# DRL-Navigation/DDRL4NAV

Measured on AMD Instinct MI355X. Metric: env-steps/sec (whole node) + PPO update ms, Pong 256 envs at 1/2/4/8 GPUs, higher is better.
Workload: dtype f32 (f16x3 MFMA planes, fp32 accumulate)

## Files before the change

ddrl4nav_amd/csrc/engine2.h:

```cpp
#pragma once
#include "kernels.h"

namespace ddrl {

using f32x16 = __attribute__((ext_vector_type(16))) float;
using f4 = __attribute__((ext_vector_type(4))) float;
using f2 = __attribute__((ext_vector_type(2))) float;
__device__ __forceinline__ f4 ld4(const float* p) { return *(const f4*)p; }
__device__ __forceinline__ void st4(float* p, f4 v) { *(f4*)p = v; }
__device__ __forceinline__ f4 zero4() { return (f4){0.0f, 0.0f, 0.0f, 0.0f}; }
typedef __attribute__((address_space(1))) const void gvoid_t;
typedef __attribute__((address_space(3))) void lvoid_t;
__device__ __forceinline__ void ld16_to_lds(const void* uniform_base, uint32_t lane_bytes, float* lds_wave_base) {
  __builtin_amdgcn_global_load_lds((gvoid_t*)((const char*)uniform_base + lane_bytes), (lvoid_t*)lds_wave_base, 16, 0, 0);
}
__device__ __forceinline__ int wave_u() { return __builtin_amdgcn_readfirstlane((int)(threadIdx.x >> 6)); }
template <int NJ>
__device__ __forceinline__ void direct_copy(const void* uniform_base, const uint32_t (&off)[NJ], float* tile, int wave, int tid, int nquads) {
#pragma unroll
  for (int j = 0; j < NJ; ++j)
    if (256 * (j + 1) <= nquads || tid + 256 * j < nquads) ld16_to_lds(uniform_base, off[j], tile + (64 * wave + 256 * j) * 4);
}
template <int N>
__device__ __forceinline__ void wait_vmcnt() {
  asm volatile("s_waitcnt vmcnt(%0)" ::"n"(N) : "memory");
}
__device__ __forceinline__ void rare_path() { asm volatile("; rare path"); }
__device__ __forceinline__ void st1_so(void* uniform_base, uint32_t lane_bytes, float v) {
  *(float*)((char*)uniform_base + lane_bytes) = v;
}

__device__ __forceinline__ float leaky_f(float v) { return __builtin_fmaxf(v, v * LEAKY); }
__device__ __forceinline__ float leaky_bit(unsigned mask, int bit, float g) {
// ... 87 lines not shown
  }
  __syncthreads();
}

template <class Op>
__global__ __launch_bounds__(Op::THREADS, 1) void engine2_kernel(typename Op::Params P) {
  extern __shared__ __attribute__((aligned(16))) float lds2[];
  Op op;
  const int tid = threadIdx.x;
  op.init(P, tid, lds2);
  typename Op::Regs regs;
  f32x16 acc[Op::TM][Op::TN];
#pragma unroll
  for (int i = 0; i < Op::TM; ++i)
#pragma unroll
    for (int j = 0; j < Op::TN; ++j)
#pragma unroll
      for (int r = 0; r < 16; ++r) acc[i][j][r] = 0.0f;

  int kb = op.kb_begin;
  const int kbe = op.kb_end;
  if (kb < kbe) {
    op.fetch(P, kb, regs);
    op.commit(regs, lds2);
    if (kb + 1 < kbe) op.fetch(P, kb + 1, regs);
  }
  __syncthreads();
  for (; kb + 2 < kbe; kb += 2) {
    engine2_step<Op, 0>(op, P, kb, kbe, regs, acc, lds2);
    engine2_step<Op, 1>(op, P, kb + 1, kbe, regs, acc, lds2);
  }
  for (int rbuf = 0; kb < kbe; ++kb, rbuf ^= 1) engine2_step<Op, -1>(op, P, kb, kbe, regs, acc, lds2, rbuf);
  op.epilogue(P, acc, lds2);
}

template <auto Kernel>
inline void lds_limit_once(int bytes) {
  static bool configured = false;
  if (!configured) {
    (void)hipFuncSetAttribute((const void*)Kernel, hipFuncAttributeMaxDynamicSharedMemorySize, bytes);
    configured = true;
  }
}

template <class Op>
inline void launch_engine2(dim3 grid, const typename Op::Params& p, hipStream_t st) {
  constexpr size_t bytes = (size_t)(2 * Op::STAGE) * sizeof(float);
  if (bytes > 64 * 1024) lds_limit_once<engine2_kernel<Op>>((int)bytes);
  hipLaunchKernelGGL(engine2_kernel<Op>, grid, dim3(Op::THREADS), bytes, st, p);
}

__device__ __forceinline__ float lane_swap1(float v) {
  return __int_as_float(__builtin_amdgcn_update_dpp(0, __float_as_int(v), 0xB1, 0xF, 0xF, true));
}

__device__ __forceinline__ int acc_row(int r, int hi) { return (r & 3) + 8 * (r >> 2) + 4 * hi; }

using f16x2_t = __attribute__((ext_vector_type(2))) _Float16;
using h8v = __attribute__((ext_vector_type(8))) _Float16;
constexpr int NPL = 2, NPROD = 3;
using frag8 = h8v;
constexpr int PA[NPROD] = {1, 0, 0}, PB[NPROD] = {0, 1, 0};
using f32x2_t = __attribute__((ext_vector_type(2))) float;
__device__ __forceinline__ void split_planes_c(float x, float y, float scale, unsigned (&p)[NPL]) {
  const f32x2_t xs = {x * scale, y * scale};
  const f16x2_t a = __builtin_convertvector(xs, f16x2_t);
// ... 61 lines not shown
```

ddrl4nav_amd/csrc/fc2.hip:

```cpp
#include "engine2.h"

namespace ddrl {



struct FcFwdB {
  static constexpr int PITCH = 80, PLANE = 128 * PITCH, B_OFF = NPL * PLANE, LDS_BYTES = 2 * NPL * PLANE;
};

template <bool SPLIT>
__global__ __launch_bounds__(256) void fc_fwd_planes_kernel(const float* __restrict__ a3, int64_t a3_es, const unsigned short* __restrict__ wlb,
                                                            const float* __restrict__ amax, const float* __restrict__ params, int64_t bias_off0,
                                                            int64_t bias_off1, float* __restrict__ h, int64_t h_es, int n, int ne, int nsplit,
                                                            float* __restrict__ part, const float* __restrict__ smax, int smax_es) {
  using K = FcFwdB;
  extern __shared__ __attribute__((aligned(16))) char ldsf[];
  const int tid = threadIdx.x, lane = tid & 63, wave = tid >> 6, l31 = lane & 31, hi = lane >> 5;
  const int wr = wave >> 1, wc = wave & 1;
  int bx = blockIdx.x, by = blockIdx.y, bz = blockIdx.z;
  if (!SPLIT && (gridDim.y & 7) == 0) {
    const int lin = bx + 4 * by, xcd = lin & 7, q = lin >> 3;
    bx = q & 3, by = (q >> 2) * 8 + xcd;
  }
  if (SPLIT) {
    const int G = 4 * (int)gridDim.y, nz = (int)gridDim.z, lin = bx + 4 * by + G * bz, full = (nz & ~7) * G;
    int g, m;
    if (lin < full) {
      const int xcd = lin & 7, r = lin >> 3;
      g = (r / G) * 8 + xcd, m = r % G;
    } else {
      const int l2 = lin - full, xcd = l2 & 7, rest = nz & 7;
      if (rest == 4) {
        g = (nz & ~7) + (xcd >> 1), m = (l2 >> 3) * 2 + (xcd & 1);
      } else {
        g = (nz & ~7) + l2 / G, m = l2 % G;
      }
    }
    bz = g, bx = m & 3, by = m >> 2;
  }
  const int e = SPLIT ? bz % ne : bz, split = SPLIT ? bz / ne : 0, n0 = bx * 128, b0 = by * 128;
  float sa = plane_scale(amax[amax_idx(AMAX_A3, e)]), inv = 1.0f / (sa * plane_scale(amax[amax_idx(AMAX_WL, e)]));
  const int k4 = tid & 7, rr = tid >> 3;
  const float* asrc[4];
#pragma unroll
  for (int j = 0; j < 4; ++j) asrc[j] = a3 + e * a3_es + (int64_t)min(b0 + rr + 32 * j, n - 1) * FLAT + k4 * 4;
  const int k8 = tid & 3, cc = tid >> 2;
  const unsigned short* wsrc = wlb + (int64_t)e * PLANE_ROOM * FLAT * FEAT + (int64_t)(n0 + cc) * FLAT + k8 * 8;
  int aA[2], bB[2];
#pragma unroll
  for (int i = 0; i < 2; ++i) aA[i] = (wr * 64 + i * 32 + l31) * K::PITCH + hi * 16;
#pragma unroll
  for (int j = 0; j < 2; ++j) bB[j] = K::B_OFF + (wc * 64 + j * 32 + l31) * K::PITCH + hi * 16;
  constexpr int DEPTH = SPLIT ? 4 : 1;
  f4 ar[DEPTH][4], wrg[DEPTH][2][NPL];
  auto fetch = [&](int kb, int slot) {
#pragma unroll
    for (int j = 0; j < 4; ++j) ar[slot][j] = ld4(asrc[j] + kb * 32);
#pragma unroll
    for (int j = 0; j < 2; ++j)
#pragma unroll
      for (int p = 0; p < NPL; ++p) wrg[slot][j][p] = *(const f4*)(wsrc + (int64_t)p * FLAT * FEAT + (int64_t)j * 64 * FLAT + kb * 32);
  };
  auto commit = [&](int slot) {
#pragma unroll
    for (int j = 0; j < 4; ++j) {
      const f4 v = ar[slot][j];
      unsigned pa[NPL], pb[NPL];
      split_planes_c(v.x, v.y, sa, pa);
      split_planes_c(v.z, v.w, sa, pb);
      char* d = ldsf + (rr + 32 * j) * K::PITCH + k4 * 8;
#pragma unroll
      for (int p = 0; p < NPL; ++p) *(uint2*)(d + p * K::PLANE) = make_uint2(pa[p], pb[p]);
    }
#pragma unroll
    for (int j = 0; j < 2; ++j)
#pragma unroll
      for (int p = 0; p < NPL; ++p) *(f4*)(ldsf + K::B_OFF + p * K::PLANE + (cc + 64 * j) * K::PITCH + k8 * 16) = wrg[slot][j][p];
  };
  f32x16 acc[2][2];
#pragma unroll
  for (int i = 0; i < 2; ++i)
#pragma unroll
    for (int j = 0; j < 2; ++j)
#pragma unroll
      for (int r = 0; r < 16; ++r) acc[i][j][r] = 0.0f;
  auto compute = [&]() {
#pragma unroll
    for (int kg = 0; kg < 2; ++kg) {
      frag8 a[NPL][2], b[NPL][2];
#pragma unroll
      for (int p = 0; p < NPL; ++p) {
#pragma unroll
        for (int i = 0; i < 2; ++i) a[p][i] = *(const frag8*)(ldsf + aA[i] + p * K::PLANE + kg * 32);
#pragma unroll
        for (int j = 0; j < 2; ++j) b[p][j] = *(const frag8*)(ldsf + bB[j] + p * K::PLANE + kg * 32);
      }
#pragma unroll
      for (int t = 0; t < NPROD; ++t)
#pragma unroll
        for (int i = 0; i < 2; ++i)
#pragma unroll
          for (int j = 0; j < 2; ++j) acc[i][j] = mfma_planes(a[PA[t]][i], b[PB[t]][j], acc[i][j]);
    }
  };
  if constexpr (SPLIT) {
    constexpr int PER = (FLAT / 32) / FC_ACT_SPLITS;
    const int kb0 = split * PER;
#pragma unroll
    for (int d = 0; d < DEPTH && d < PER; ++d) fetch(kb0 + d, d);
    if (smax != nullptr) {
      float m = 0.0f;
      for (int i = tid; i < n; i += 256) m = fmaxf(m, smax[e * smax_es + i]);
      m = wave_fmax(m);
      float* red = (float*)ldsf;
      if (lane == 0) red[wave] = m;
      __syncthreads();
      const float a3top = fmaxf(fmaxf(red[0], red[1]), fmaxf(red[2], red[3]));
      __syncthreads();
      sa = plane_scale(a3top), inv = 1.0f / (sa * plane_scale(amax[amax_idx(AMAX_WL, e)]));
    }
    commit(0);
    if (DEPTH < PER) fetch(kb0 + DEPTH, 0);
    __syncthreads();
#pragma unroll
    for (int k = 0; k < PER; ++k) {
      compute();
      __syncthreads();
      if (k + 1 < PER) {
        commit((k + 1) % DEPTH);
        if (k + 1 + DEPTH < PER) fetch(kb0 + k + 1 + DEPTH, (k + 1) % DEPTH);
      }
      __syncthreads();
    }
  } else {
    constexpr int NKB = FLAT / 32;
    fetch(0, 0);
    commit(0);
    fetch(1, 0);
    __syncthreads();
    for (int kb = 0; kb < NKB; ++kb) {
      compute();
      __syncthreads();
      if (kb + 1 < NKB) {
        commit(0);
        if (kb + 2 < NKB) fetch(kb + 2, 0);
      }
      __syncthreads();
    }
  }
#pragma unroll
  for (int j = 0; j < 2; ++j) {
    const int nn = n0 + wc * 64 + j * 32 + l31;
    const float bias = SPLIT ? 0.0f : params[(e ? bias_off1 : bias_off0) + nn];
    float* dst = SPLIT ? part + ((int64_t)split * ENC_SLOTS + e) * n * FEAT : h + e * h_es;
#pragma unroll
    for (int i = 0; i < 2; ++i)
#pragma unroll
      for (int r = 0; r < 16; ++r) {
        const int b = b0 + wr * 64 + i * 32 + acc_row(r, hi);
        if (b < n) dst[(int64_t)b * FEAT + nn] = acc[i][j][r] * inv + bias;
      }
  }
}

void launch_fc_forward(const EncCall& c, bool allow_split, hipStream_t st, bool per_sample_max) {
  const Workspace& w = *c.ws;
  const int nsplit = allow_split ? fc_forward_splits(c.n) : 1;
  ProfRange pr(c.prof, nsplit > 1 ? "FcFwdSplit" : "FcFwd", st);
  {
    lds_limit_once<fc_fwd_planes_kernel<false>>((int)FcFwdB::LDS_BYTES);
    lds_limit_once<fc_fwd_planes_kernel<true>>((int)FcFwdB::LDS_BYTES);
    const dim3 grid(FEAT / 128, (c.n + 127) / 128, c.L->NE * nsplit);
    if (nsplit > 1)
      hipLaunchKernelGGL(fc_fwd_planes_kernel<true>, grid, dim3(256), FcFwdB::LDS_BYTES, st, w.a3, w.es(A3_N), w.wlb, w.amax, c.params,
                         c.L->enc_base[0] + c.L->enc.lb, c.L->enc_base[c.L->NE - 1] + c.L->enc.lb, w.h, w.es(H_N), c.n, c.L->NE, nsplit, w.wpart,
                         per_sample_max ? w.actmax : (const float*)nullptr, ACT_FUSED_MAX);
    else
      hipLaunchKernelGGL(fc_fwd_planes_kernel<false>, grid, dim3(256), FcFwdB::LDS_BYTES, st, w.a3, w.es(A3_N), w.wlb, w.amax, c.params,
                         c.L->enc_base[0] + c.L->enc.lb, c.L->enc_base[c.L->NE - 1] + c.L->enc.lb, w.h, w.es(H_N), c.n, c.L->NE, 1, w.wpart,
                         (const float*)nullptr, 0);
  }
}

struct FcDgradB {
  static constexpr int KBK = 32, WPE = 2, PITCH = 2 * KBK + 16, PLANE = 128 * PITCH, B_OFF = NPL * PLANE, LDS_BYTES = 2 * NPL * PLANE;
  static constexpr int NAQ = KBK / 4, ARJ = 128 * NAQ / 256, AROWS = 256 / NAQ;
  static constexpr int NWF = KBK / 8, WJ = 128 * NWF / 256, WCOLS = 256 / NWF;
};
__global__ __launch_bounds__(256) __attribute__((amdgpu_waves_per_eu(FcDgradB::WPE, FcDgradB::WPE))) void fc_dgrad_planes_kernel(const float* __restrict__ dh, int64_t dh_es, const unsigned short* __restrict__ wdlb,
                                                              float* __restrict__ amax, const unsigned* __restrict__ m3, float* __restrict__ dz3, int64_t a3_es, int n) {
  using K = FcDgradB;
  extern __shared__ __attribute__((aligned(16))) char ldsg[];
  const int tid = threadIdx.x, lane = tid & 63, wave = tid >> 6, l31 = lane & 31, hi = lane >> 5;
  const int wr = wave >> 1, wc = wave & 1;
  int bx = blockIdx.x, by = blockIdx.y;
  if ((gridDim.y & 7) == 0) {
    const int lin = bx + 25 * by, xcd = lin & 7, q = lin >> 3;
    if ((gridDim.y & 63) != 0) {
      bx = q % 25, by = (q / 25) * 8 + xcd;
    } else {
      const int blk = q / 40, r = q % 40;
      bx = (blk % 5) * 5 + r % 5, by = ((blk / 5) * 8 + r / 5) * 8 + xcd;
    }
  }
  const int e = blockIdx.z, k0 = bx * 128, b0 = by * 128;
  const float sa = plane_scale(amax[amax_idx(AMAX_DH, e)]), inv = 1.0f / (sa * plane_scale(amax[amax_idx(AMAX_WL, e)]));
  const int n4 = tid % K::NAQ, rr = tid / K::NAQ;
  const float* asrc[K::ARJ];
#pragma unroll
  for (int j = 0; j < K::ARJ; ++j) asrc[j] = dh + e * dh_es + (int64_t)min(b0 + rr + K::AROWS * j, n - 1) * FEAT + n4 * 4;
  const int n8 = tid % K::NWF, cc = tid / K::NWF;
  const unsigned short* wsrc[K::WJ];
#pragma unroll
  for (int j = 0; j < K::WJ; ++j) wsrc[j] = wdlb + (int64_t)e * PLANE_ROOM * FLAT * FEAT + (int64_t)min(k0 + cc + K::WCOLS * j, FLAT - 1) * FEAT + n8 * 8;
  int aA[2], bB[2];
#pragma unroll
  for (int i = 0; i < 2; ++i) aA[i] = (wr * 64 + i * 32 + l31) * K::PITCH + hi * 16;
#pragma unroll
  for (int j = 0; j < 2; ++j) bB[j] = K::B_OFF + (wc * 64 + j * 32 + l31) * K::PITCH + hi * 16;
  f4 ar[K::ARJ], wrg[K::WJ][NPL];
  auto fetch = [&](int kb) {
#pragma unroll
    for (int j = 0; j < K::ARJ; ++j) ar[j] = ld4(asrc[j] + kb * K::KBK);
#pragma unroll
    for (int j = 0; j < K::WJ; ++j)
#pragma unroll
      for (int p = 0; p < NPL; ++p) wrg[j][p] = *(const f4*)(wsrc[j] + (int64_t)p * FLAT * FEAT + kb * K::KBK);
  };
  auto commit = [&]() {
#pragma unroll
    for (int j = 0; j < K::ARJ; ++j) {
      const f4 v = ar[j];
      unsigned pa[NPL], pb[NPL];
      split_planes_c(v.x, v.y, sa, pa);
      split_planes_c(v.z, v.w, sa, pb);
      char* d = ldsg + (rr + K::AROWS * j) * K::PITCH + n4 * 8;
#pragma unroll
      for (int p = 0; p < NPL; ++p) *(uint2*)(d + p * K::PLANE) = make_uint2(pa[p], pb[p]);
    }
#pragma unroll
    for (int j = 0; j < K::WJ; ++j)
#pragma unroll
      for (int p = 0; p < NPL; ++p) *(f4*)(ldsg + K::B_OFF + p * K::PLANE + (cc + K::WCOLS * j) * K::PITCH + n8 * 16) = wrg[j][p];
  };
  f32x16 acc[2][2];
#pragma unroll
  for (int i = 0; i < 2; ++i)
#pragma unroll
    for (int j = 0; j < 2; ++j)
#pragma unroll
      for (int r = 0; r < 16; ++r) acc[i][j][r] = 0.0f;
  constexpr int NKB = FEAT / K::KBK;
  fetch(0);
  commit();
  fetch(1);
  __syncthreads();
  for (int kb = 0; kb < NKB; ++kb) {
#pragma unroll
    for (int kg = 0; kg < K::KBK / 16; ++kg) {
      frag8 a[NPL][2], b[NPL][2];
#pragma unroll
      for (int p = 0; p < NPL; ++p) {
#pragma unroll
        for (int i = 0; i < 2; ++i) a[p][i] = *(const frag8*)(ldsg + aA[i] + p * K::PLANE + kg * 32);
#pragma unroll
        for (int j = 0; j < 2; ++j) b[p][j] = *(const frag8*)(ldsg + bB[j] + p * K::PLANE + kg * 32);
      }
#pragma unroll
      for (int t = 0; t < NPROD; ++t)
#pragma unroll
        for (int i = 0; i < 2; ++i)
#pragma unroll
          for (int j = 0; j < 2; ++j) acc[i][j] = mfma_planes(a[PA[t]][i], b[PB[t]][j], acc[i][j]);
    }
    __syncthreads();
    if (kb + 1 < NKB) {
      commit();
      if (kb + 2 < NKB) fetch(kb + 2);
    }
    __syncthreads();
  }
  float big = 0.0f;
#pragma unroll
  for (int j = 0; j < 2; ++j) {
    const int k = k0 + wc * 64 + j * 32 + l31;
    if (k >= FLAT) continue;
    const int ch = k / 49, pix = k % 49;
    const int mbit = 16 * (ch >> 5) + 15 - ((ch & 3) + 4 * ((ch & 31) >> 3));
    const unsigned* mp = m3 + (int64_t)e * (a3_es / A3_N) * M3_N + pix * 2 + ((ch >> 2) & 1);
#pragma unroll
    for (int i = 0; i < 2; ++i) {
      unsigned mw[16];
#pragma unroll
      for (int r = 0; r < 16; ++r) {
        const int b = min(b0 + wr * 64 + i * 32 + acc_row(r, hi), n - 1);
        mw[r] = mp[(int64_t)b * M3_N];
      }
#pragma unroll
      for (int r = 0; r < 16; ++r) {
        const int b = b0 + wr * 64 + i * 32 + acc_row(r, hi);
        const float g = leaky_bit(mw[r], mbit, acc[i][j][r] * inv);
        if (b < n) {
          dz3[e * a3_es + (int64_t)b * FLAT + k] = g;
          big = fmaxf(big, fabsf(g));
        }
      }
    }
  }
  amax_update(big, amax + amax_idx(AMAX_DZ3, e));
}

struct FcWgradB {
  static constexpr int KB = 32, PITCH = 320, PLANE = KB * PITCH, B_OFF = NPL * PLANE, LDS_BYTES = 2 * NPL * PLANE;
  static constexpr int64_t SLAB = SLAB_FC;
};

__global__ __launch_bounds__(256) void fc_wgrad_planes_kernel(const float* __restrict__ dh, int64_t dh_es, const float* __restrict__ a3,
                                                              int64_t a3_es, const float* __restrict__ amax, const float* __restrict__ gsc,
                                                              int64_t gsc_es, float* __restrict__ part, int n, int nsplit, int ne) {
  using K = FcWgradB;
  extern __shared__ __attribute__((aligned(16))) char ldsw[];
  const int tid = threadIdx.x, lane = tid & 63, wave = tid >> 6, l31 = lane & 31, hi = lane >> 5;
  const int wr = wave >> 1, wc = wave & 1;
  const int unit = (int)(blockIdx.x >> 5) * 8 + (int)(blockIdx.x & 7);
  if (unit >= 25 * ne * nsplit) return;
  const int bx = unit % 25, by = (int)(blockIdx.x >> 3) & 3, bz = unit / 25;
  const int e = bz % ne, split = bz / ne;
  const float sd = WGRAD_HEADROOM * plane_scale(amax[amax_idx(AMAX_DH, e)]) / amax[amax_idx(AMAX_GMAX, e)], sa = plane_scale(amax[amax_idx(AMAX_A3, e)]),
              inv = 1.0f / (sd * sa);
  const float* gs = gsc + e * gsc_es;
  const int k0 = bx * 128, n0 = by * 128;
  const int nkb = (n + K::KB - 1) / K::KB;
  const int per = (nkb + nsplit - 1) / nsplit;
  const int kb_begin = split * per, kb_end = min(nkb, kb_begin + per);
  const int c4 = tid & 31, kk = tid >> 5;
  const float* dsrc = dh + e * dh_es + n0 + c4 * 4;
  const float* asrc = a3 + e * a3_es + min(k0 + c4 * 4, FLAT - 4);
  const int g16 = lane >> 4, q = (lane >> 2) & 3, pp = lane & 3;
  int aA[2], bB[2];
#pragma unroll
  for (int i = 0; i < 2; ++i) aA[i] = (8 * (g16 >> 1) + q) * K::PITCH + (wr * 64 + i * 32 + 16 * (g16 & 1) + 4 * pp) * 2;
#pragma unroll
  for (int j = 0; j < 2; ++j) bB[j] = K::B_OFF + (8 * (g16 >> 1) + q) * K::PITCH + (wc * 64 + j * 32 + 16 * (g16 & 1) + 4 * pp) * 2;
  f4 dr[4], ar[4];
  float gr[4];
  f4 bsum = zero4();
  const bool bias_owner = (bx == 0);
  auto fetch = [&](int kb) {
#pragma unroll
    for (int j = 0; j < 4; ++j) {
      const int64_t row = min(kb * K::KB + kk + 8 * j, n - 1);
      dr[j] = ld4(dsrc + row * FEAT);
      ar[j] = ld4(asrc + row * FLAT);
      gr[j] = gs[row];
    }
  };
  auto commit = [&](int kb) {
    if (kb * K::KB + K::KB > n) {
      rare_path();
#pragma unroll
      for (int j = 0; j < 4; ++j)
        if (kb * K::KB + kk + 8 * j >= n) dr[j] = zero4();
      rare_path();
    }
#pragma unroll
    for (int j = 0; j < 4; ++j) {
      char* d = ldsw + (kk + 8 * j) * K::PITCH + c4 * 8;
      unsigned pa[NPL], pb[NPL];
      const float sdj = sd * gr[j];
      split_planes(dr[j].x, dr[j].y, sdj, pa);
      split_planes(dr[j].z, dr[j].w, sdj, pb);
#pragma unroll
      for (int p = 0; p < NPL; ++p) *(uint2*)(d + p * K::PLANE) = make_uint2(pa[p], pb[p]);
      split_planes(ar[j].x, ar[j].y, sa, pa);
      split_planes(ar[j].z, ar[j].w, sa, pb);
#pragma unroll
      for (int p = 0; p < NPL; ++p) *(uint2*)(d + K::B_OFF + p * K::PLANE) = make_uint2(pa[p], pb[p]);
    }
    if (bias_owner) bsum += (dr[0] * gr[0] + dr[1] * gr[1]) + (dr[2] * gr[2] + dr[3] * gr[3]);
  };
  f32x16 acc[2][2];
#pragma unroll
  for (int i = 0; i < 2; ++i)
#pragma unroll
    for (int j = 0; j < 2; ++j)
#pragma unroll
      for (int r = 0; r < 16; ++r) acc[i][j][r] = 0.0f;
  if (kb_begin < kb_end) {
    fetch(kb_begin);
    commit(kb_begin);
    if (kb_begin + 1 < kb_end) fetch(kb_begin + 1);
    __syncthreads();
    for (int kb = kb_begin; kb < kb_end; ++kb) {
#pragma unroll
      for (int kg = 0; kg < 2; ++kg) {
        frag8 a[NPL][2], b[NPL][2];
#pragma unroll
        for (int p = 0; p < NPL; ++p) {
          const int off = p * K::PLANE + kg * 16 * K::PITCH;
#pragma unroll
          for (int i = 0; i < 2; ++i) a[p][i] = tr_frag(ldsw, aA[i] + off, aA[i] + off + 4 * K::PITCH);
#pragma unroll
          for (int j = 0; j < 2; ++j) b[p][j] = tr_frag(ldsw, bB[j] + off, bB[j] + off + 4 * K::PITCH);
        }
#pragma unroll
        for (int t = 0; t < NPROD; ++t)
#pragma unroll
          for (int i = 0; i < 2; ++i)
#pragma unroll
            for (int j = 0; j < 2; ++j) acc[i][j] = mfma_planes(a[PA[t]][i], b[PB[t]][j], acc[i][j]);
      }
      __syncthreads();
      if (kb + 1 < kb_end) {
        commit(kb + 1);
        if (kb + 2 < kb_end) fetch(kb + 2);
      }
      __syncthreads();
    }
  }
  float* slab = part + ((int64_t)split * ENC_SLOTS + e) * K::SLAB;
#pragma unroll
  for (int j = 0; j < 2; ++j) {
    const int k = k0 + wc * 64 + j * 32 + l31;
    if (k >= FLAT) continue;
#pragma unroll
    for (int i = 0; i < 2; ++i)
#pragma unroll
      for (int r = 0; r < 16; ++r) slab[(int64_t)(n0 + wr * 64 + i * 32 + acc_row(r, hi)) * FLAT + k] = acc[i][j][r] * inv;
  }
  if (bias_owner) {
    float* red = (float*)ldsw;
    st4(red + kk * 128 + c4 * 4, bsum);
    __syncthreads();
    if (tid < 128) {
      float s = 0.0f;
#pragma unroll
      for (int t = 0; t < 8; ++t) s += red[t * 128 + tid];
      slab[(int64_t)FEAT * FLAT + n0 + tid] = s;
    }
  }
}

void launch_fc_backward(const EncCall& c, float* grads, hipStream_t st, int part) {
  const Workspace& w = *c.ws;
  const ParamLayout& L = *c.L;
  const int S = c.splits->fc;
  if (part != 1) {
    {
// ... 19 lines not shown
```

ddrl4nav_amd/csrc/wgrad2.hip:

```cpp
#include <type_traits>

#include "engine2.h"

namespace ddrl {


__device__ __forceinline__ float ld_gs(const float* gs, int idx) {
  asm volatile("" : "+v"(idx));
  return gs[idx];
}

template <int I, int N, class F>
__device__ __forceinline__ void static_for(F&& f) {
  if constexpr (I < N) {
    f(std::integral_constant<int, I>{});
    static_for<I + 1, N>(f);
  }
}

struct WgradSplit {
  int pair_begin, pair_end;
  __device__ __forceinline__ void set(int n, int nsplit, int split) {
    const int npairs = (n + 1) >> 1;
    const int per = (npairs + nsplit - 1) / nsplit;
    pair_begin = min(npairs, split * per);
    pair_end = min(npairs, pair_begin + per);
  }
};

using u4w = __attribute__((ext_vector_type(4))) unsigned;

struct Wgrad3P {
  static constexpr int BP = 64;
  static constexpr int WPE = 1;
  static constexpr int KAP0 = 48, KAP1 = 50, NKG0 = 3, NKG1 = 4;
  static constexpr int PX0 = 81, PX1 = 27 + 81;
  static constexpr int A_PLANE0 = NKG0 * 16 * 128, A_PLANE1 = NKG1 * 16 * 128;
  static constexpr int B_HALF0 = PX0 * BP, B_HALF1 = PX1 * BP, B_PLANE0 = 2 * B_HALF0, B_PLANE1 = 2 * B_HALF1;
  static constexpr int A0 = 0, B0 = A0 + NPL * A_PLANE0, A1 = B0 + NPL * B_PLANE0, B1 = A1 + NPL * A_PLANE1;
  static constexpr int LDS_BYTES = B1 + NPL * B_PLANE1;
  static constexpr int AU0 = KAP0 * 8, AU1 = KAP1 * 8, BU0 = PX0 * 8, BU1 = PX1 * 8;
  static constexpr int NA = 2, NB0 = 3, NB1 = 4;
  static_assert(AU0 <= 256 * NA && AU1 <= 256 * NA && BU0 <= 256 * NB0 && BU1 <= 256 * NB1 && NB0 + 1 == NB1, "units per thread");
  static_assert(LDS_BYTES <= 160 * 1024, "LDS budget");
  static_assert(98 * 8 * 8 * 4 <= LDS_BYTES, "the bias reduction reuses the buffers");
  static constexpr int WG_PER_CU = (WPE >= 2 && LDS_BYTES <= 80 * 1024) ? 2 : 1;
  static constexpr int64_t SLAB = SLAB3;
};

__global__ __launch_bounds__(256, Wgrad3P::WPE) void conv_wgrad3_pipe_kernel(const float* __restrict__ a2, int64_t a2_es, const float* __restrict__ dz3,
// ... 695 lines not shown
```

Measured before the change: 257,200.

## Double-buffer LDS and interleave staging with MFMA in FC forward, dgrad, wgrad

Reworks the three FC plane-GEMM kernels (non-split forward, dgrad, wgrad) to use two LDS stages instead of one. Global fetch, plane split and LDS commit for the next k-block are issued in units between MFMA blocks, with sched_group_barrier hints to interleave them. This drops one __syncthreads per k-step and hides global and LDS latency behind matrix math. The cost is twice the LDS and more register pressure, with occupancy pinned via waves_per_eu, and the forward kernel is split into separate SPLIT and non-split specializations.

Result: no change. 259,000, median of 6 (+0.7%).

```diff
diff --git a/ddrl4nav_amd/csrc/engine2.h b/ddrl4nav_amd/csrc/engine2.h
--- a/ddrl4nav_amd/csrc/engine2.h
+++ b/ddrl4nav_amd/csrc/engine2.h
@@ -1,4 +1,6 @@
 #pragma once
+#include <type_traits>
+
 #include "kernels.h"
 
 namespace ddrl {
@@ -152,6 +154,14 @@
   }
   for (int rbuf = 0; kb < kbe; ++kb, rbuf ^= 1) engine2_step<Op, -1>(op, P, kb, kbe, regs, acc, lds2, rbuf);
   op.epilogue(P, acc, lds2);
+}
+
+template <int I, int N, class F>
+__device__ __forceinline__ void static_for(F&& f) {
+  if constexpr (I < N) {
+    f(std::integral_constant<int, I>{});
+    static_for<I + 1, N>(f);
+  }
 }
 
 template <auto Kernel>
diff --git a/ddrl4nav_amd/csrc/fc2.hip b/ddrl4nav_amd/csrc/fc2.hip
--- a/ddrl4nav_amd/csrc/fc2.hip
+++ b/ddrl4nav_amd/csrc/fc2.hip
@@ -3,13 +3,78 @@
 namespace ddrl {
 
 
+
+template <class K, int BUF, int STG, class Fetch, class Commit>
+__device__ __forceinline__ void fc_pipe_step(const char* lds, const int (&aA)[2], const int (&bB)[2], f32x16 (&acc)[2][2], Fetch& fetch_unit,
+                                             Commit& commit_unit, int kb) {
+  const char* cur = lds + BUF * K::STAGE;
+  frag8 a[2][NPL][2], b[2][NPL][2];
+  auto read_frags = [&](int kg, frag8 (&fa)[NPL][2], frag8 (&fb)[NPL][2]) __attribute__((always_inline)) {
+#pragma unroll
+    for (int p = 0; p < NPL; ++p) {
+#pragma unroll
+      for (int i = 0; i < 2; ++i) fa[p][i] = *(const frag8*)(cur + aA[i] + p * K::PLANE + kg * 32);
+#pragma unroll
+      for (int j = 0; j < 2; ++j) fb[p][j] = *(const frag8*)(cur + bB[j] + p * K::PLANE + kg * 32);
+    }
+  };
+  read_frags(0, a[0], b[0]);
+  static_for<0, K::NBLK>([&](auto bc) __attribute__((always_inline)) {
+    constexpr int blk = decltype(bc)::value, kg = blk / NPROD, t = blk % NPROD;
+    constexpr bool ahead = t == 0 && kg + 1 < K::NKG;
+    if constexpr (ahead) read_frags(kg + 1, a[(kg + 1) & 1], b[(kg + 1) & 1]);
+#pragma unroll
+    for (int i = 0; i < 2; ++i)
+#pragma unroll
+      for (int j = 0; j < 2; ++j) acc[i][j] = mfma_planes(a[kg & 1][PA[t]][i], b[kg & 1][PB[t]][j], acc[i][j]);
+    if constexpr (STG >= 1) commit_unit(bc, BUF ^ 1);
+    if constexpr (STG >= 2) fetch_unit(bc, kb + 2);
+    constexpr int PIN = 4;
+    if constexpr (blk == 0) __builtin_amdgcn_sched_group_barrier(0x100, 4 * NPL, 0);
+#pragma unroll
+    for (int m = 0; m < 4; ++m) {
+      __builtin_amdgcn_sched_group_barrier(0x008, 1, 0);
+      if constexpr (ahead) __builtin_amdgcn_sched_group_barrier(0x100, NPL, 0);
+      if constexpr (STG >= 1) __builtin_amdgcn_sched_group_barrier(0x002, PIN, 0);
+    }
+    if constexpr (STG >= 2) __builtin_amdgcn_sched_group_barrier(0x020, NPL, 0);
+    if constexpr (STG >= 1) __builtin_amdgcn_sched_group_barrier(0x200, NPL, 0);
+    __builtin_amdgcn_sched_barrier(0);
+  });
+}
+
+template <class K, int NKB, class Fetch, class Commit>
+__device__ __forceinline__ void fc_pipe_loop(const char* lds, const int (&aA)[2], const int (&bB)[2], f32x16 (&acc)[2][2], Fetch& fetch_unit,
+                                             Commit& commit_unit) {
+  static_assert(K::NU == K::NBLK, "one staging unit per MFMA block");
+  static_assert(NKB % 2 == 0 && NKB >= 4, "the k loop is unrolled by the two stages");
+  static_for<0, K::NU>([&](auto uc) __attribute__((always_inline)) { fetch_unit(uc, 0); });
+  static_for<0, K::NU>([&](auto uc) __attribute__((always_inline)) { commit_unit(uc, 0); });
+  static_for<0, K::NU>([&](auto uc) __attribute__((always_inline)) { fetch_unit(uc, 1); });
+  __syncthreads();
+  for (int kb = 0; kb < NKB - 2; kb += 2) {
+    fc_pipe_step<K, 0, 2>(lds, aA, bB, acc, fetch_unit, commit_unit, kb);
+    __syncthreads();
+    fc_pipe_step<K, 1, 2>(lds, aA, bB, acc, fetch_unit, commit_unit, kb + 1);
+    __syncthreads();
+  }
+  fc_pipe_step<K, 0, 1>(lds, aA, bB, acc, fetch_unit, commit_unit, NKB - 2);
+  __syncthreads();
+  fc_pipe_step<K, 1, 0>(lds, aA, bB, acc, fetch_unit, commit_unit, NKB - 1);
+}
 
 struct FcFwdB {
   static constexpr int PITCH = 80, PLANE = 128 * PITCH, B_OFF = NPL * PLANE, LDS_BYTES = 2 * NPL * PLANE;
 };
 
 template <bool SPLIT>
-__global__ __launch_bounds__(256) void fc_fwd_planes_kernel(const float* __restrict__ a3, int64_t a3_es, const unsigned short* __restrict__ wlb,
+__global__ void fc_fwd_planes_kernel(const float* __restrict__ a3, int64_t a3_es, const unsigned short* __restrict__ wlb,
+                                                            const float* __restrict__ amax, const float* __restrict__ params, int64_t bias_off0,
+                                                            int64_t bias_off1, float* __restrict__ h, int64_t h_es, int n, int ne, int nsplit,
+                                                            float* __restrict__ part, const float* __restrict__ smax, int smax_es);
+
+template <>
+__global__ __launch_bounds__(256) void fc_fwd_planes_kernel<true>(const float* __restrict__ a3, int64_t a3_es, const unsigned short* __restrict__ wlb,
                                                             const float* __restrict__ amax, const float* __restrict__ params, int64_t bias_off0,
                                                             int64_t bias_off1, float* __restrict__ h, int64_t h_es, int n, int ne, int nsplit,
                                                             float* __restrict__ part, const float* __restrict__ smax, int smax_es) {
@@ -18,27 +83,21 @@
   const int tid = threadIdx.x, lane = tid & 63, wave = tid >> 6, l31 = lane & 31, hi = lane >> 5;
   const int wr = wave >> 1, wc = wave & 1;
   int bx = blockIdx.x, by = blockIdx.y, bz = blockIdx.z;
-  if (!SPLIT && (gridDim.y & 7) == 0) {
-    const int lin = bx + 4 * by, xcd = lin & 7, q = lin >> 3;
-    bx = q & 3, by = (q >> 2) * 8 + xcd;
-  }
-  if (SPLIT) {
-    const int G = 4 * (int)gridDim.y, nz = (int)gridDim.z, lin = bx + 4 * by + G * bz, full = (nz & ~7) * G;
-    int g, m;
-    if (lin < full) {
-      const int xcd = lin & 7, r = lin >> 3;
-      g = (r / G) * 8 + xcd, m = r % G;
+  const int G = 4 * (int)gridDim.y, nz = (int)gridDim.z, lin = bx + 4 * by + G * bz, full = (nz & ~7) * G;
+  int g, m;
+  if (lin < full) {
+    const int xcd = lin & 7, r = lin >> 3;
+    g = (r / G) * 8 + xcd, m = r % G;
+  } else {
+    const int l2 = lin - full, xcd = l2 & 7, rest = nz & 7;
+    if (rest == 4) {
+      g = (nz & ~7) + (xcd >> 1), m = (l2 >> 3) * 2 + (xcd & 1);
     } else {
-      const int l2 = lin - full, xcd = l2 & 7, rest = nz & 7;
-      if (rest == 4) {
-        g = (nz & ~7) + (xcd >> 1), m = (l2 >> 3) * 2 + (xcd & 1);
-      } else {
-        g = (nz & ~7) + l2 / G, m = l2 % G;
-      }
-    }
-    bz = g, bx = m & 3, by = m >> 2;
-  }
-  const int e = SPLIT ? bz % ne : bz, split = SPLIT ? bz / ne : 0, n0 = bx * 128, b0 = by * 128;
+      g = (nz & ~7) + l2 / G, m = l2 % G;
+    }
+  }
+  bz = g, bx = m & 3, by = m >> 2;
+  const int e = bz % ne, split = bz / ne, n0 = bx * 128, b0 = by * 128;
   float sa = plane_scale(amax[amax_idx(AMAX_A3, e)]), inv = 1.0f / (sa * plane_scale(amax[amax_idx(AMAX_WL, e)]));
   const int k4 = tid & 7, rr = tid >> 3;
   const float* asrc[4];
@@ -51,7 +110,7 @@
   for (int i = 0; i < 2; ++i) aA[i] = (wr * 64 + i * 32 + l31) * K::PITCH + hi * 16;
 #pragma unroll
   for (int j = 0; j < 2; ++j) bB[j] = K::B_OFF + (wc * 64 + j * 32 + l31) * K::PITCH + hi * 16;
-  constexpr int DEPTH = SPLIT ? 4 : 1;
+  constexpr int DEPTH = 4;
   f4 ar[DEPTH][4], wrg[DEPTH][2][NPL];
   auto fetch = [&](int kb, int slot) {
 #pragma unroll
@@ -103,56 +162,121 @@
           for (int j = 0; j < 2; ++j) acc[i][j] = mfma_planes(a[PA[t]][i], b[PB[t]][j], acc[i][j]);
     }
   };
-  if constexpr (SPLIT) {
-    constexpr int PER = (FLAT / 32) / FC_ACT_SPLITS;
-    const int kb0 = split * PER;
-#pragma unroll
-    for (int d = 0; d < DEPTH && d < PER; ++d) fetch(kb0 + d, d);
-    if (smax != nullptr) {
-      float m = 0.0f;
-      for (int i = tid; i < n; i += 256) m = fmaxf(m, smax[e * smax_es + i]);
-      m = wave_fmax(m);
-      float* red = (float*)ldsf;
-      if (lane == 0) red[wave] = m;
-      __syncthreads();
-      const float a3top = fmaxf(fmaxf(red[0], red[1]), fmaxf(red[2], red[3]));
-      __syncthreads();
-      sa = plane_scale(a3top), inv = 1.0f / (sa * plane_scale(amax[amax_idx(AMAX_WL, e)]));
-    }
-    commit(0);
-    if (DEPTH < PER) fetch(kb0 + DEPTH, 0);
-    __syncthreads();
-#pragma unroll
-    for (int k = 0; k < PER; ++k) {
-      compute();
-      __syncthreads();
-      if (k + 1 < PER) {
-        commit((k + 1) % DEPTH);
-        if (k + 1 + DEPTH < PER) fetch(kb0 + k + 1 + DEPTH, (k + 1) % DEPTH);
-      }
-      __syncthreads();
-    }
-  } else {
-    constexpr int NKB = FLAT / 32;
-    fetch(0, 0);
-    commit(0);
-    fetch(1, 0);
-    __syncthreads();
-    for (int kb = 0; kb < NKB; ++kb) {
-      compute();
-      __syncthreads();
-      if (kb + 1 < NKB) {
-        commit(0);
-        if (kb + 2 < NKB) fetch(kb + 2, 0);
-      }
-      __syncthreads();
-    }
+  constexpr int PER = (FLAT / 32) / FC_ACT_SPLITS;
+  const int kb0 = split * PER;
+#pragma unroll
+  for (int d = 0; d < DEPTH && d < PER; ++d) fetch(kb0 + d, d);
+  if (smax != nullptr) {
+    float m = 0.0f;
+    for (int i = tid; i < n; i += 256) m = fmaxf(m, smax[e * smax_es + i]);
+    m = wave_fmax(m);
+    float* red = (float*)ldsf;
+    if (lane == 0) red[wave] = m;
+    __syncthreads();
+    const float a3top = fmaxf(fmaxf(red[0], red[1]), fmaxf(red[2], red[3]));
+    __syncthreads();
+    sa = plane_scale(a3top), inv = 1.0f / (sa * plane_scale(amax[amax_idx(AMAX_WL, e)]));
+  }
+  commit(0);
+  if (DEPTH < PER) fetch(kb0 + DEPTH, 0);
+  __syncthreads();
+#pragma unroll
+  for (int k = 0; k < PER; ++k) {
+    compute();
+    __syncthreads();
+    if (k + 1 < PER) {
+      commit((k + 1) % DEPTH);
+      if (k + 1 + DEPTH < PER) fetch(kb0 + k + 1 + DEPTH, (k + 1) % DEPTH);
+    }
+    __syncthreads();
   }
 #pragma unroll
   for (int j = 0; j < 2; ++j) {
     const int nn = n0 + wc * 64 + j * 32 + l31;
-    const float bias = SPLIT ? 0.0f : params[(e ? bias_off1 : bias_off0) + nn];
-    float* dst = SPLIT ? part + ((int64_t)split * ENC_SLOTS + e) * n * FEAT : h + e * h_es;
+    float* dst = part + ((int64_t)split * ENC_SLOTS + e) * n * FEAT;
+#pragma unroll
+    for (int i = 0; i < 2; ++i)
+#pragma unroll
+      for (int r = 0; r < 16; ++r) {
+        const int b = b0 + wr * 64 + i * 32 + acc_row(r, hi);
+        if (b < n) dst[(int64_t)b * FEAT + nn] = acc[i][j][r] * inv + 0.0f;
+      }
+  }
+}
+
+struct FcFwdP {
+  static constexpr int WPE = 2, PITCH = FcFwdB::PITCH, PLANE = FcFwdB::PLANE, B_OFF = FcFwdB::B_OFF, STAGE = FcFwdB::LDS_BYTES, LDS_BYTES = 2 * STAGE;
+  static constexpr int ARJ = 4, WJ = 2, NKG = 2, NBLK = NKG * NPROD, NU = ARJ + WJ;
+  static_assert(LDS_BYTES <= 80 * 1024, "two workgroups per CU");
+};
+template <>
+__global__ __launch_bounds__(256) __attribute__((amdgpu_waves_per_eu(FcFwdP::WPE, FcFwdP::WPE))) void fc_fwd_planes_kernel<false>(const float* __restrict__ a3, int64_t a3_es, const unsigned short* __restrict__ wlb,
+                                                            const float* __restrict__ amax, const float* __restrict__ params, int64_t bias_off0,
+                                                            int64_t bias_off1, float* __restrict__ h, int64_t h_es, int n, int ne, int nsplit,
+                                                            float* __restrict__ part, const float* __restrict__ smax, int smax_es) {
+  using K = FcFwdP;
+  extern __shared__ __attribute__((aligned(16))) char ldsp[];
+  const int tid = threadIdx.x, lane = tid & 63, wave = tid >> 6, l31 = lane & 31, hi = lane >> 5;
+  const int wr = wave >> 1, wc = wave & 1;
+  int bx = blockIdx.x, by = blockIdx.y;
+  if ((gridDim.y & 7) == 0) {
+    const int lin = bx + 4 * by, xcd = lin & 7, q = lin >> 3;
+    bx = q & 3, by = (q >> 2) * 8 + xcd;
+  }
+  const int e = blockIdx.z, n0 = bx * 128, b0 = by * 128;
+  const float sa = plane_scale(amax[amax_idx(AMAX_A3, e)]), inv = 1.0f / (sa * plane_scale(amax[amax_idx(AMAX_WL, e)]));
+  const int k4 = tid & 7, rr = tid >> 3;
+  const float* asrc[K::ARJ];
+#pragma unroll
+  for (int j = 0; j < K::ARJ; ++j) asrc[j] = a3 + e * a3_es + (int64_t)min(b0 + rr + 32 * j, n - 1) * FLAT + k4 * 4;
+  const int k8 = tid & 3, cc = tid >> 2;
+  const unsigned short* wsrc = wlb + (int64_t)e * PLANE_ROOM * FLAT * FEAT + (int64_t)(n0 + cc) * FLAT + k8 * 8;
+  int aA[2], bB[2];
+#pragma unroll
+  for (int i = 0; i < 2; ++i) aA[i] = (wr * 64 + i * 32 + l31) * K::PITCH + hi * 16;
+#pragma unroll
+  for (int j = 0; j < 2; ++j) bB[j] = K::B_OFF + (wc * 64 + j * 32 + l31) * K::PITCH + hi * 16;
+  f4 ar[K::ARJ], wrg[K::WJ][NPL];
+  auto fetch_unit = [&](auto uc, int kb) __attribute__((always_inline)) {
+    constexpr int u = decltype(uc)::value;
+    if constexpr (u < K::ARJ) {
+      ar[u] = ld4(asrc[u] + kb * 32);
+    } else {
+      constexpr int j = u - K::ARJ;
+#pragma unroll
+      for (int p = 0; p < NPL; ++p) wrg[j][p] = *(const f4*)(wsrc + (int64_t)p * FLAT * FEAT + (int64_t)j * 64 * FLAT + kb * 32);
+    }
+  };
+  auto commit_unit = [&](auto uc, int buf) __attribute__((always_inline)) {
+    constexpr int u = decltype(uc)::value;
+    char* stage = ldsp + buf * K::STAGE;
+    if constexpr (u < K::ARJ) {
+      const f4 v = ar[u];
+      unsigned pa[NPL], pb[NPL];
+      split_planes_c(v.x, v.y, sa, pa);
+      split_planes_c(v.z, v.w, sa, pb);
+      char* d = stage + (rr + 32 * u) * K::PITCH + k4 * 8;
+#pragma unroll
+      for (int p = 0; p < NPL; ++p) *(uint2*)(d + p * K::PLANE) = make_uint2(pa[p], pb[p]);
+    } else {
+      constexpr int j = u - K::ARJ;
+#pragma unroll
+      for (int p = 0; p < NPL; ++p) *(f4*)(stage + K::B_OFF + p * K::PLANE + (cc + 64 * j) * K::PITCH + k8 * 16) = wrg[j][p];
+    }
+  };
+  f32x16 acc[2][2];
+#pragma unroll
+  for (int i = 0; i < 2; ++i)
+#pragma unroll
+    for (int j = 0; j < 2; ++j)
+#pragma unroll
+      for (int r = 0; r < 16; ++r) acc[i][j][r] = 0.0f;
+  fc_pipe_loop<K, FLAT / 32>(ldsp, aA, bB, acc, fetch_unit, commit_unit);
+#pragma unroll
+  for (int j = 0; j < 2; ++j) {
+    const int nn = n0 + wc * 64 + j * 32 + l31;
+    const float bias = params[(e ? bias_off1 : bias_off0) + nn];
+    float* dst = h + e * h_es;
 #pragma unroll
     for (int i = 0; i < 2; ++i)
 #pragma unroll
@@ -168,7 +292,7 @@
   const int nsplit = allow_split ? fc_forward_splits(c.n) : 1;
   ProfRange pr(c.prof, nsplit > 1 ? "FcFwdSplit" : "FcFwd", st);
   {
-    lds_limit_once<fc_fwd_planes_kernel<false>>((int)FcFwdB::LDS_BYTES);
+    lds_limit_once<fc_fwd_planes_kernel<false>>((int)FcFwdP::LDS_BYTES);
     lds_limit_once<fc_fwd_planes_kernel<true>>((int)FcFwdB::LDS_BYTES);
     const dim3 grid(FEAT / 128, (c.n + 127) / 128, c.L->NE * nsplit);
     if (nsplit > 1)
@@ -176,16 +300,18 @@
                          c.L->enc_base[0] + c.L->enc.lb, c.L->enc_base[c.L->NE - 1] + c.L->enc.lb, w.h, w.es(H_N), c.n, c.L->NE, nsplit, w.wpart,
                          per_sample_max ? w.actmax : (const float*)nullptr, ACT_FUSED_MAX);
     else
-      hipLaunchKernelGGL(fc_fwd_planes_kernel<false>, grid, dim3(256), FcFwdB::LDS_BYTES, st, w.a3, w.es(A3_N), w.wlb, w.amax, c.params,
+      hipLaunchKernelGGL(fc_fwd_planes_kernel<false>, grid, dim3(256), FcFwdP::LDS_BYTES, st, w.a3, w.es(A3_N), w.wlb, w.amax, c.params,
                          c.L->enc_base[0] + c.L->enc.lb, c.L->enc_base[c.L->NE - 1] + c.L->enc.lb, w.h, w.es(H_N), c.n, c.L->NE, 1, w.wpart,
                          (const float*)nullptr, 0);
   }
 }
 
 struct FcDgradB {
-  static constexpr int KBK = 32, WPE = 2, PITCH = 2 * KBK + 16, PLANE = 128 * PITCH, B_OFF = NPL * PLANE, LDS_BYTES = 2 * NPL * PLANE;
+  static constexpr int KBK = 32, WPE = 2, PITCH = 2 * KBK + 16, PLANE = 128 * PITCH, B_OFF = NPL * PLANE, STAGE = 2 * NPL * PLANE, LDS_BYTES = 2 * STAGE;
   static constexpr int NAQ = KBK / 4, ARJ = 128 * NAQ / 256, AROWS = 256 / NAQ;
   static constexpr int NWF = KBK / 8, WJ = 128 * NWF / 256, WCOLS = 256 / NWF;
+  static constexpr int NKG = KBK / 16, NBLK = NKG * NPROD, NU = ARJ + WJ;
+  static_assert(LDS_BYTES <= 80 * 1024, "two workgroups per CU");
 };
 __global__ __launch_bounds__(256) __attribute__((amdgpu_waves_per_eu(FcDgradB::WPE, FcDgradB::WPE))) void fc_dgrad_planes_kernel(const float* __restrict__ dh, int64_t dh_es, const unsigned short* __restrict__ wdlb,
                                                               float* __restrict__ amax, const unsigned* __restrict__ m3, float* __restrict__ dz3, int64_t a3_es, int n) {
@@ -219,29 +345,32 @@
 #pragma unroll
   for (int j = 0; j < 2; ++j) bB[j] = K::B_OFF + (wc * 64 + j * 32 + l31) * K::PITCH + hi * 16;
   f4 ar[K::ARJ], wrg[K::WJ][NPL];
-  auto fetch = [&](int kb) {
-#pragma unroll
-    for (int j = 0; j < K::ARJ; ++j) ar[j] = ld4(asrc[j] + kb * K::KBK);
-#pragma unroll
-    for (int j = 0; j < K::WJ; ++j)
+  auto fetch_unit = [&](auto uc, int kb) __attribute__((always_inline)) {
+    constexpr int u = decltype(uc)::value;
+    if constexpr (u < K::ARJ) {
+      ar[u] = ld4(asrc[u] + kb * K::KBK);
+    } else {
+      constexpr int j = u - K::ARJ;
 #pragma unroll
       for (int p = 0; p < NPL; ++p) wrg[j][p] = *(const f4*)(wsrc[j] + (int64_t)p * FLAT * FEAT + kb * K::KBK);
-  };
-  auto commit = [&]() {
-#pragma unroll
-    for (int j = 0; j < K::ARJ; ++j) {
-      const f4 v = ar[j];
+    }
+  };
+  auto commit_unit = [&](auto uc, int buf) __attribute__((always_inline)) {
+    constexpr int u = decltype(uc)::value;
+    char* stage = ldsg + buf * K::STAGE;
+    if constexpr (u < K::ARJ) {
+      const f4 v = ar[u];
       unsigned pa[NPL], pb[NPL];
       split_planes_c(v.x, v.y, sa, pa);
       split_planes_c(v.z, v.w, sa, pb);
-      char* d = ldsg + (rr + K::AROWS * j) * K::PITCH + n4 * 8;
+      char* d = stage + (rr + K::AROWS * u) * K::PITCH + n4 * 8;
 #pragma unroll
       for (int p = 0; p < NPL; ++p) *(uint2*)(d + p * K::PLANE) = make_uint2(pa[p], pb[p]);
-    }
-#pragma unroll
-    for (int j = 0; j < K::WJ; ++j)
-#pragma unroll
-      for (int p = 0; p < NPL; ++p) *(f4*)(ldsg + K::B_OFF + p * K::PLANE + (cc + K::WCOLS * j) * K::PITCH + n8 * 16) = wrg[j][p];
+    } else {
+      constexpr int j = u - K::ARJ;
+#pragma unroll
+      for (int p = 0; p < NPL; ++p) *(f4*)(stage + K::B_OFF + p * K::PLANE + (cc + K::WCOLS * j) * K::PITCH + n8 * 16) = wrg[j][p];
+    }
   };
   f32x16 acc[2][2];
 #pragma unroll
@@ -250,36 +379,7 @@
     for (int j = 0; j < 2; ++j)
 #pragma unroll
       for (int r = 0; r < 16; ++r) acc[i][j][r] = 0.0f;
-  constexpr int NKB = FEAT / K::KBK;
-  fetch(0);
-  commit();
-  fetch(1);
-  __syncthreads();
-  for (int kb = 0; kb < NKB; ++kb) {
-#pragma unroll
-    for (int kg = 0; kg < K::KBK / 16; ++kg) {
-      frag8 a[NPL][2], b[NPL][2];
-#pragma unroll
-      for (int p = 0; p < NPL; ++p) {
-#pragma unroll
-        for (int i = 0; i < 2; ++i) a[p][i] = *(const frag8*)(ldsg + aA[i] + p * K::PLANE + kg * 32);
-#pragma unroll
-        for (int j = 0; j < 2; ++j) b[p][j] = *(const frag8*)(ldsg + bB[j] + p * K::PLANE + kg * 32);
-      }
-#pragma unroll
-      for (int t = 0; t < NPROD; ++t)
-#pragma unroll
-        for (int i = 0; i < 2; ++i)
-#pragma unroll
-          for (int j = 0; j < 2; ++j) acc[i][j] = mfma_planes(a[PA[t]][i], b[PB[t]][j], acc[i][j]);
-    }
-    __syncthreads();
-    if (kb + 1 < NKB) {
-      commit();
-      if (kb + 2 < NKB) fetch(kb + 2);
-    }
-    __syncthreads();
-  }
+  fc_pipe_loop<K, FEAT / K::KBK>(ldsg, aA, bB, acc, fetch_unit, commit_unit);
   float big = 0.0f;
 #pragma unroll
   for (int j = 0; j < 2; ++j) {
@@ -311,11 +411,14 @@
 }
 
 struct FcWgradB {
-  static constexpr int KB = 32, PITCH = 320, PLANE = KB * PITCH, B_OFF = NPL * PLANE, LDS_BYTES = 2 * NPL * PLANE;
+  static constexpr int KB = 32, WPE = 2, PITCH = 320, PLANE = KB * PITCH, B_OFF = NPL * PLANE, STAGE = 2 * NPL * PLANE, LDS_BYTES = 2 * STAGE;
+  static constexpr int NKG = KB / 16, NBLK = NKG * NPROD, NU = 4;
+  static_assert(NU + 2 <= NBLK, "units ride on MFMA blocks 1 .. NU");
+  static_assert(LDS_BYTES <= 80 * 1024, "two workgroups per CU");
   static constexpr int64_t SLAB = SLAB_FC;
 };
 
-__global__ __launch_bounds__(256) void fc_wgrad_planes_kernel(const float* __restrict__ dh, int64_t dh_es, const float* __restrict__ a3,
+__global__ __launch_bounds__(256) __attribute__((amdgpu_waves_per_eu(FcWgradB::WPE, FcWgradB::WPE))) void fc_wgrad_planes_kernel(const float* __restrict__ dh, int64_t dh_es, const float* __restrict__ a3,
                                                               int64_t a3_es, const float* __restrict__ amax, const float* __restrict__ gsc,
                                                               int64_t gsc_es, float* __restrict__ part, int n, int nsplit, int ne) {
   using K = FcWgradB;
@@ -342,42 +445,50 @@
   for (int i = 0; i < 2; ++i) aA[i] = (8 * (g16 >> 1) + q) * K::PITCH + (wr * 64 + i * 32 + 16 * (g16 & 1) + 4 * pp) * 2;
 #pragma unroll
   for (int j = 0; j < 2; ++j) bB[j] = K::B_OFF + (8 * (g16 >> 1) + q) * K::PITCH + (wc * 64 + j * 32 + 16 * (g16 & 1) + 4 * pp) * 2;
-  f4 dr[4], ar[4];
-  float gr[4];
+  f4 dr[K::NU], ar[K::NU], pr[K::NU];
+  float gr[K::NU];
   f4 bsum = zero4();
   const bool bias_owner = (bx == 0);
-  auto fetch = [&](int kb) {
-#pragma unroll
-    for (int j = 0; j < 4; ++j) {
-      const int64_t row = min(kb * K::KB + kk + 8 * j, n - 1);
-      dr[j] = ld4(dsrc + row * FEAT);
-      ar[j] = ld4(asrc + row * FLAT);
-      gr[j] = gs[row];
-    }
-  };
-  auto commit = [&](int kb) {
+  auto fetch_unit = [&](auto uc, int kb) __attribute__((always_inline)) {
+    constexpr int j = decltype(uc)::value;
+    const int64_t row = min(kb * K::KB + kk + 8 * j, n - 1);
+    dr[j] = ld4(dsrc + row * FEAT);
+    ar[j] = ld4(asrc + row * FLAT);
+    gr[j] = gs[row];
+  };
+  auto mask = [&](int kb) __attribute__((always_inline)) {
     if (kb * K::KB + K::KB > n) {
       rare_path();
 #pragma unroll
-      for (int j = 0; j < 4; ++j)
+      for (int j = 0; j < K::NU; ++j)
         if (kb * K::KB + kk + 8 * j >= n) dr[j] = zero4();
       rare_path();
     }
-#pragma unroll
-    for (int j = 0; j < 4; ++j) {
-      char* d = ldsw + (kk + 8 * j) * K::PITCH + c4 * 8;
-      unsigned pa[NPL], pb[NPL];
-      const float sdj = sd * gr[j];
-      split_planes(dr[j].x, dr[j].y, sdj, pa);
+  };
+  auto commit_part = [&](auto uc, auto mc, char* stage, unsigned (&pa)[NPL], unsigned (&pb)[NPL]) __attribute__((always_inline)) {
+    constexpr int j = decltype(uc)::value, m = decltype(mc)::value;
+    char* d = stage + (kk + 8 * j) * K::PITCH + c4 * 8;
+    const float sdj = sd * gr[j];
+    if constexpr (m == 0) split_planes(dr[j].x, dr[j].y, sdj, pa);
+    if constexpr (m == 1) {
       split_planes(dr[j].z, dr[j].w, sdj, pb);
 #pragma unroll
       for (int p = 0; p < NPL; ++p) *(uint2*)(d + p * K::PLANE) = make_uint2(pa[p], pb[p]);
-      split_planes(ar[j].x, ar[j].y, sa, pa);
+    }
+    if constexpr (m == 2) split_planes(ar[j].x, ar[j].y, sa, pa);
+    if constexpr (m == 3) {
       split_planes(ar[j].z, ar[j].w, sa, pb);
 #pragma unroll
       for (int p = 0; p < NPL; ++p) *(uint2*)(d + K::B_OFF + p * K::PLANE) = make_uint2(pa[p], pb[p]);
-    }
-    if (bias_owner) bsum += (dr[0] * gr[0] + dr[1] * gr[1]) + (dr[2] * gr[2] + dr[3] * gr[3]);
+      pr[j] = dr[j] * gr[j];
+    }
+  };
+  auto commit_unit = [&](auto uc, char* stage) __attribute__((always_inline)) {
+    unsigned pa[NPL], pb[NPL];
+    static_for<0, 4>([&](auto mc) __attribute__((always_inline)) { commit_part(uc, mc, stage, pa, pb); });
+  };
+  auto bias_add = [&]() __attribute__((always_inline)) {
+    if (bias_owner) bsum += (pr[0] + pr[1]) + (pr[2] + pr[3]);
   };
   f32x16 acc[2][2];
 #pragma unroll
@@ -386,23 +497,72 @@
     for (int j = 0; j < 2; ++j)
 #pragma unroll
       for (int r = 0; r < 16; ++r) acc[i][j][r] = 0.0f;
+  auto read_frags = [&](const char* cur, int kg, frag8 (&fa)[NPL][2], frag8 (&fb)[NPL][2]) __attribute__((always_inline)) {
+#pragma unroll
+    for (int p = 0; p < NPL; ++p) {
+      const int off = p * K::PLANE + kg * 16 * K::PITCH;
+#pragma unroll
+      for (int i = 0; i < 2; ++i) fa[p][i] = tr_frag(cur, aA[i] + off, aA[i] + off + 4 * K::PITCH);
+#pragma unroll
+      for (int j = 0; j < 2; ++j) fb[p][j] = tr_frag(cur, bB[j] + off, bB[j] + off + 4 * K::PITCH);
+    }
+  };
+  auto step = [&](auto bufc, int kb) __attribute__((always_inline)) {
+    constexpr int BUF = decltype(bufc)::value;
+    const char* cur = ldsw + BUF * K::STAGE;
+    mask(kb + 1);
+    frag8 a[2][NPL][2], b[2][NPL][2];
+    read_frags(cur, 0, a[0], b[0]);
+    static_for<0, K::NBLK>([&](auto bc) __attribute__((always_inline)) {
+      constexpr int blk = decltype(bc)::value, kg = blk / NPROD, t = blk % NPROD;
+      constexpr bool ahead = t == 0 && kg + 1 < K::NKG, staged = blk >= 1 && blk <= K::NU;
+      if constexpr (ahead) read_frags(cur, kg + 1, a[(kg + 1) & 1], b[(kg + 1) & 1]);
+      if constexpr (staged) {
+        using U = std::integral_constant<int, blk - 1>;
+        unsigned pa[NPL], pb[NPL];
+        static_for<0, 4>([&](auto mc) __attribute__((always_inline)) {
+          constexpr int m = decltype(mc)::value, i = m >> 1, j = m & 1;
+          acc[i][j] = mfma_planes(a[kg & 1][PA[t]][i], b[kg & 1][PB[t]][j], acc[i][j]);
+          commit_part(U{}, mc, ldsw + (BUF ^ 1) * K::STAGE, pa, pb);
+          if constexpr (m == 3) fetch_unit(U{}, kb + 2);
+          __builtin_amdgcn_sched_barrier(0);
+        });
+      } else {
+#pragma unroll
+        for (int i = 0; i < 2; ++i)
+#pragma unroll
+          for (int j = 0; j < 2; ++j) acc[i][j] = mfma_planes(a[kg & 1][PA[t]][i], b[kg & 1][PB[t]][j], acc[i][j]);
+        if constexpr (blk == 0) __builtin_amdgcn_sched_group_barrier(0x100, 8 * NPL, 0);
+#pragma unroll
+        for (int m = 0; m < 4; ++m) {
+          __builtin_amdgcn_sched_group_barrier(0x008, 1, 0);
+          if constexpr (ahead) __builtin_amdgcn_sched_group_barrier(0x100, 2 * NPL, 0);
+        }
+        __builtin_amdgcn_sched_barrier(0);
+      }
+    });
+    bias_add();
+  };
   if (kb_begin < kb_end) {
-    fetch(kb_begin);
-    commit(kb_begin);
-    if (kb_begin + 1 < kb_end) fetch(kb_begin + 1);
-    __syncthreads();
-    for (int kb = kb_begin; kb < kb_end; ++kb) {
-#pragma unroll
-      for (int kg = 0; kg < 2; ++kg) {
+    static_for<0, K::NU>([&](auto uc) __attribute__((always_inline)) { fetch_unit(uc, kb_begin); });
+    mask(kb_begin);
+    static_for<0, K::NU>([&](auto uc) __attribute__((always_inline)) { commit_unit(uc, ldsw); });
+    bias_add();
+    if (kb_begin + 1 < kb_end) static_for<0, K::NU>([&](auto uc) __attribute__((always_inline)) { fetch_unit(uc, kb_begin + 1); });
+    __syncthreads();
+    int kb = kb_begin;
+    for (; kb + 3 < kb_end; kb += 2) {
+      step(std::integral_constant<int, 0>{}, kb);
+      __syncthreads();
+      step(std::integral_constant<int, 1>{}, kb + 1);
+      __syncthreads();
+    }
+    for (int buf = 0; kb < kb_end; ++kb, buf ^= 1) {
+      const char* cur = ldsw + buf * K::STAGE;
+#pragma unroll
+      for (int kg = 0; kg < K::NKG; ++kg) {
         frag8 a[NPL][2], b[NPL][2];
-#pragma unroll
-        for (int p = 0; p < NPL; ++p) {
-          const int off = p * K::PLANE + kg * 16 * K::PITCH;
-#pragma unroll
-          for (int i = 0; i < 2; ++i) a[p][i] = tr_frag(ldsw, aA[i] + off, aA[i] + off + 4 * K::PITCH);
-#pragma unroll
-          for (int j = 0; j < 2; ++j) b[p][j] = tr_frag(ldsw, bB[j] + off, bB[j] + off + 4 * K::PITCH);
-        }
+        read_frags(cur, kg, a, b);
 #pragma unroll
         for (int t = 0; t < NPROD; ++t)
 #pragma unroll
@@ -410,10 +570,11 @@
 #pragma unroll
             for (int j = 0; j < 2; ++j) acc[i][j] = mfma_planes(a[PA[t]][i], b[PB[t]][j], acc[i][j]);
       }
-      __syncthreads();
       if (kb + 1 < kb_end) {
-        commit(kb + 1);
-        if (kb + 2 < kb_end) fetch(kb + 2);
+        mask(kb + 1);
+        static_for<0, K::NU>([&](auto uc) __attribute__((always_inline)) { commit_unit(uc, ldsw + (buf ^ 1) * K::STAGE); });
+        bias_add();
+        if (kb + 2 < kb_end) static_for<0, K::NU>([&](auto uc) __attribute__((always_inline)) { fetch_unit(uc, kb + 2); });
       }
       __syncthreads();
     }
diff --git a/ddrl4nav_amd/csrc/wgrad2.hip b/ddrl4nav_amd/csrc/wgrad2.hip
--- a/ddrl4nav_amd/csrc/wgrad2.hip
+++ b/ddrl4nav_amd/csrc/wgrad2.hip
@@ -1,5 +1,3 @@
-#include <type_traits>
-
 #include "engine2.h"
 
 namespace ddrl {
@@ -8,14 +6,6 @@
 __device__ __forceinline__ float ld_gs(const float* gs, int idx) {
   asm volatile("" : "+v"(idx));
   return gs[idx];
-}
-
-template <int I, int N, class F>
-__device__ __forceinline__ void static_for(F&& f) {
-  if constexpr (I < N) {
-    f(std::integral_constant<int, I>{});
-    static_for<I + 1, N>(f);
-  }
 }
 
 struct WgradSplit {
```
